# hyunlord/hnm_recommendation

Measured on AMD Instinct MI355X. Metric: recommendations/sec (batched users, K=12) at 1/2/4/8 MI355X; % HBM roofline, higher is better.
Workload: dtype f16+f32; 1 GPU; ncf: BASELINE configs[1] NeuralCF dim=64, full H&M shape, batch=4096 users/rank, K=12; users=1371980, items=105542, batch_per_rank=4096, k=12, parallelism=single, model=NeuralCF, mf_dim=64, weights=init, scan=certified f16 pre-filter + exact fp32 re-scoring (ncf_cert.hip)

## Files before the change

hnm_recommendation_amd/_lib.py:

```python
from __future__ import annotations

import ctypes as C
import os
import threading
import weakref

import torch

PKG = os.path.dirname(os.path.abspath(__file__))
LIB_PATH = os.environ.get("HNM_LIB_PATH") or os.path.join(PKG, "libhnm_mi355x.so")

HNM_OK, HNM_EINVAL, HNM_EOOB, HNM_EHIP, HNM_ENOMEM, HNM_EUNSUPPORTED, HNM_ECOLL = 0, -1, -2, -3, -4, -5, -6

_p = C.c_void_p
_i64 = C.c_int64
_i32 = C.c_int32
_f32 = C.c_float


class NcfWeights(C.Structure):
    _fields_ = [("gmf_user", _p), ("gmf_item", _p), ("mlp_user", _p), ("mlp_item", _p),
                ("w1", _p), ("b1", _p), ("w2", _p), ("b2", _p), ("wp", _p), ("bp", _p),
                ("num_users", _i64), ("num_items", _i64), ("mf", _i32), ("h0", _i32),
                ("h1", _i32), ("h2", _i32), ("item_proj", _p)]
# ... 160 lines not shown
        if _lib is not None:
            return _lib
        if not os.path.exists(path):
            raise RuntimeError(
                f"{path} is missing: the MI355X HIP library was not built "
                "(run `python -m hnm_recommendation_amd.build`). There is no CPU fallback.")
        lib = C.CDLL(path)
        for name, (res, args) in _SIGS.items():
            fn = getattr(lib, name, None)
            if fn is None:
                continue
            fn.restype = res
            fn.argtypes = args
        if lib.hnm_abi_version() != 1:
            raise RuntimeError("libhnm_mi355x ABI version mismatch")
        _lib = lib
        return lib


def fn(name):
    lib = load()
    f = getattr(lib, name, None)
    if f is None:
        raise RuntimeError(f"{name} is not exported by {LIB_PATH}")
    return f


def check(status: int, what: str = ""):
    if status == HNM_OK:
        return
    msg = load().hnm_last_error().decode(errors="replace")
    if status == HNM_EOOB:
        raise IndexError(msg)
    if status in (HNM_EINVAL, HNM_EUNSUPPORTED):
        raise ValueError(f"{what}: {msg}")
    raise RuntimeError(f"{what}: {msg} (status {status})")


def call(name: str, *args):
    check(fn(name)(*args), name)


def call_weighted(name: str, at: int, w, *args):
    if w is not None:
        name, args = name.replace("_f32", "_weighted_f32"), (*args[:at], ptr(w), *args[at:])
    check(fn(name)(*args), name)


def require_gpu(*tensors):
    for t in tensors:
        if t is None:
            continue
        on_gpu = t.type == "cuda" if isinstance(t, torch.device) else (
            isinstance(t, torch.Tensor) and t.is_cuda)
        if not on_gpu:
            raise RuntimeError(
                "hnm_recommendation_amd runs on an AMD Instinct GPU (MI355X) through its HIP "
                "library; move the module and its inputs to a GPU device (model.to('cuda')). "
                "There is no CPU path.")


def _dev_index(device) -> int:
    dev = torch.device(device)
    return dev.index if dev.index is not None else torch.cuda.current_device()


_opts: dict = {}


class _Ctx:
    __slots__ = ("handle", "device", "__weakref__")

    def __init__(self, device: int):
        h = _p()
        check(fn("hnm_ctx_create")(device, C.byref(h)), "hnm_ctx_create")
        self.handle, self.device = h, device

    def __del__(self):
        h, self.handle = self.handle, None
        lib = _lib
        if h and lib is not None:
            try:
                lib.hnm_ctx_destroy(h)
            except Exception:
                pass


def _thread_ctx(idx: int) -> "_Ctx":
    slots = getattr(_tls, "ctxs", None)
    if slots is None:
        slots = _tls.ctxs = {}
    c = slots.get(idx)
    if c is None:
        c = _Ctx(idx)
        with _lock:
            for opt, val in _opts.get(idx, {}).items():
                check(fn("hnm_ctx_set_option")(c.handle, int(opt), int(val)), "hnm_ctx_set_option")
            _live.add(c)
        slots[idx] = c
    return c


def _device_ctxs(idx: int):
    with _lock:
        return [c for c in list(_live) if c.device == idx and c.handle]


def live_contexts(device=None) -> int:
    if device is None:
        with _lock:
            return sum(1 for c in list(_live) if c.handle)
    return len(_device_ctxs(_dev_index(device)))


def ctx(device: torch.device):
    idx = _dev_index(device)
    c = _thread_ctx(idx)
    stream = torch.cuda.current_stream(idx).cuda_stream
    check(fn("hnm_ctx_set_stream")(c.handle, _p(stream)), "hnm_ctx_set_stream")
    return c.handle


def abort_pending(device):
    check(fn("hnm_ctx_abort_pending")(ctx(device)), "hnm_ctx_abort_pending")


def sync_check(device):
    check(fn("hnm_ctx_check")(ctx(device)), "hnm_ctx_check")


TIME_SCORE, TIME_SPMM = 1, 2


def enable_timing(device, on=True):
    check(fn("hnm_ctx_enable_timing")(ctx(device), int(on)), "hnm_ctx_enable_timing")


def kernel_timing(device):
    t = C.c_double()
    n = _i64()
    check(fn("hnm_ctx_timing")(ctx(device), C.byref(t), C.byref(n)), "hnm_ctx_timing")
    return t.value, n.value


HNM_OPT_PREFILTER = 1
HNM_OPT_STATS = 3
HNM_OPT_STRIDED = 4
HNM_OPT_DEEP_MFMA = 5
HNM_OPT_LINEAR_MFMA = 6
HNM_OPT_NCF_TABLES = 7
HNM_OPT_SCAN_SHAPE = 8
HNM_OPT_SCAN_PIPE = 9
HNM_OPT_SCAN_SPARSE = 10


def set_option(device, option, value):
    idx = _dev_index(device)
    ctx(device)
    with _lock:
        _opts.setdefault(idx, {})[int(option)] = int(value)
    for c in _device_ctxs(idx):
        check(fn("hnm_ctx_set_option")(c.handle, int(option), int(value)), "hnm_ctx_set_option")


def set_prefilter(device, on=True):
    set_option(device, HNM_OPT_PREFILTER, int(bool(on)))


def prefilter_stats(device, reset=False, extended=False):
    ctx(device)
    n = {"gate": 6, "cascade": 7}.get(extended, 4) if extended else 3
    tot = [0] * n
    for c in _device_ctxs(_dev_index(device)):
        out = (_i64 * n)()
        check(fn("hnm_ctx_prefilter_stats_ex")(c.handle, out, n, int(reset)),
              "hnm_ctx_prefilter_stats_ex")
        for j in range(n):
            tot[j] += int(out[j])
    return tuple(tot)


def ptr(t):
    return None if t is None else _p(t.data_ptr())
```

hnm_recommendation_amd/csrc/api.hip:

```cpp
#include <stdlib.h>
#include <string.h>

#include "hnm_device.h"
#include "hnm_internal.h"
#include "linear_mfma.h"

static thread_local char g_err[512] = "";

void hnm_set_error(const char* fmt, ...) {
  va_list ap;
  va_start(ap, fmt);
  vsnprintf(g_err, sizeof(g_err), fmt, ap);
  va_end(ap);
}

extern "C" int hnm_abi_version(void) { return HNM_ABI_VERSION; }
extern "C" const char* hnm_last_error(void) { return g_err; }

extern "C" hnm_status hnm_ctx_create(int device, hnm_ctx** out) {
  HNM_REQUIRE(out, HNM_EINVAL, "hnm_ctx_create: out is NULL");
  int ndev = 0;
  HNM_HIP_CHECK(hipGetDeviceCount(&ndev));
  HNM_REQUIRE(device >= 0 && device < ndev, HNM_EINVAL, "hnm_ctx_create: no device %d (%d visible)",
              device, ndev);
  const HnmDeviceGuard guard(device);
  hnm_ctx* c = (hnm_ctx*)calloc(1, sizeof(hnm_ctx));
  HNM_REQUIRE(c, HNM_ENOMEM, "hnm_ctx_create: out of host memory");
  c->device = device;
  c->stream = 0;
  hipDeviceProp_t prop;
  if (hipGetDeviceProperties(&prop, device) == hipSuccess) c->num_cus = prop.multiProcessorCount;
  if (c->num_cus <= 0) c->num_cus = 256;
  c->prefilter = 1;
  c->strided = 0;
  c->deep_mfma = 1;
#ifndef HNM_LINEAR_MFMA_DEFAULT
#define HNM_LINEAR_MFMA_DEFAULT 1
#endif
  c->linear_mfma = HNM_LINEAR_MFMA_DEFAULT;
  c->ncf_tables = 1;
  c->scan_shape = 1;
  c->scan_pipe = 1;
  c->scan_sparse = 1;
  if (hipMalloc((void**)&c->err_dev, 128) != hipSuccess) {
    free(c);
    hnm_set_error("hnm_ctx_create: hipMalloc of the error word failed");
    return HNM_ENOMEM;
  }
  HNM_HIP_CHECK(hipMemset(c->err_dev, 0, 128));
  HNM_HIP_CHECK(hipEventCreateWithFlags(&c->chain_ev, hipEventDisableTiming));
  HNM_HIP_CHECK(hipStreamCreateWithFlags(&c->side, hipStreamNonBlocking));
  HNM_HIP_CHECK(hipEventCreateWithFlags(&c->side_in, hipEventDisableTiming));
  HNM_HIP_CHECK(hipEventCreateWithFlags(&c->side_out, hipEventDisableTiming));
  static_assert(8 + HNM_STATS_N * sizeof(unsigned long long) <= 128, "error word + counters");
  c->stats_dev = reinterpret_cast<unsigned long long*>(reinterpret_cast<char*>(c->err_dev) + 8);
  *out = c;
  return HNM_OK;
}

extern "C" hnm_status hnm_ctx_destroy(hnm_ctx* ctx) {
  HNM_CTX_DEVICE(ctx);
  if (!ctx) return HNM_OK;
  (void)hipDeviceSynchronize();
  for (int i = 0; i < ctx->cap; ++i) {
    (void)hipEventDestroy(ctx->ev0[i]);
    (void)hipEventDestroy(ctx->ev1[i]);
  }
  free(ctx->ev0);
  free(ctx->ev1);
  hnm_rccl_release(ctx);
  if (ctx->ws) (void)hipFree(ctx->ws);
  if (ctx->err_dev) (void)hipFree(ctx->err_dev);
  (void)hipEventDestroy(ctx->chain_ev);
  (void)hipEventDestroy(ctx->side_in);
  (void)hipEventDestroy(ctx->side_out);
  (void)hipStreamDestroy(ctx->side);
  free(ctx);
  return HNM_OK;
}

extern "C" hnm_status hnm_ctx_set_stream(hnm_ctx* ctx, void* s) {
  HNM_CTX_DEVICE(ctx);
  HNM_REQUIRE(ctx, HNM_EINVAL, "ctx is NULL");
  const hipStream_t ns = (hipStream_t)s;
  if (ns == ctx->stream) return HNM_OK;
  HNM_HIP_CHECK(hipEventRecord(ctx->chain_ev, ctx->stream));
  HNM_HIP_CHECK(hipStreamWaitEvent(ns, ctx->chain_ev, 0));
  ctx->stream = ns;
  return HNM_OK;
}

extern "C" hnm_status hnm_ctx_abort_pending(hnm_ctx* ctx) {
  HNM_CTX_DEVICE(ctx);
  HNM_REQUIRE(ctx, HNM_EINVAL, "ctx is NULL");
  ctx->pend.kind = 0;
  return HNM_OK;
}

extern "C" hnm_status hnm_ctx_set_option(hnm_ctx* ctx, int option, int64_t value) {
  HNM_CTX_DEVICE(ctx);
  HNM_REQUIRE(ctx, HNM_EINVAL, "ctx is NULL");
  switch (option) {
    case HNM_OPT_PREFILTER:
      ctx->prefilter = value != 0;
      return HNM_OK;
    case HNM_OPT_STATS:
      ctx->stats_on = value != 0;
      return HNM_OK;
    case HNM_OPT_STRIDED:
      ctx->strided = value != 0;
      return HNM_OK;
    case HNM_OPT_DEEP_MFMA:
      ctx->deep_mfma = value != 0;
      return HNM_OK;
    case HNM_OPT_LINEAR_MFMA:
      ctx->linear_mfma = value != 0;
      return HNM_OK;
    case HNM_OPT_NCF_TABLES:
      ctx->ncf_tables = value != 0;
      return HNM_OK;
    case HNM_OPT_SCAN_SHAPE:
      ctx->scan_shape = value != 0;
      return HNM_OK;
    case HNM_OPT_SCAN_PIPE:
      ctx->scan_pipe = value != 0;
      return HNM_OK;
    case HNM_OPT_SCAN_SPARSE:
      ctx->scan_sparse = value != 0;
      return HNM_OK;
    default:
      hnm_set_error("hnm_ctx_set_option: unknown option %d", option);
      return HNM_EINVAL;
  }
}

extern "C" hnm_status hnm_ctx_prefilter_stats(hnm_ctx* ctx, int64_t* out, int reset) {
  HNM_CTX_DEVICE(ctx);
  return hnm_ctx_prefilter_stats_ex(ctx, out, 3, reset);
}

extern "C" hnm_status hnm_ctx_prefilter_stats_ex(hnm_ctx* ctx, int64_t* out, int n, int reset) {
  HNM_CTX_DEVICE(ctx);
  HNM_REQUIRE(ctx && out, HNM_EINVAL, "ctx/out is NULL");
  HNM_REQUIRE(n >= 1 && n <= HNM_STATS_N, HNM_EINVAL, "prefilter_stats: 1 <= n <= %d", HNM_STATS_N);
  int prev = -1;
  HNM_HIP_CHECK(hipGetDevice(&prev));
  struct Restore {
    int dev;
    ~Restore() { (void)hipSetDevice(dev); }
  } restore{prev};
  HNM_HIP_CHECK(hipSetDevice(ctx->device));
  HNM_HIP_CHECK(hipDeviceSynchronize());
  unsigned long long v[HNM_STATS_N];
  HNM_HIP_CHECK(hipMemcpy(v, ctx->stats_dev, sizeof(v), hipMemcpyDeviceToHost));
  for (int i = 0; i < n; ++i) out[i] = (int64_t)v[i];
  if (reset) HNM_HIP_CHECK(hipMemset(ctx->stats_dev, 0, sizeof(v)));
  return HNM_OK;
}

extern "C" hnm_status hnm_ctx_num_cus(hnm_ctx* ctx, int* out) {
  HNM_CTX_DEVICE(ctx);
  HNM_REQUIRE(ctx && out, HNM_EINVAL, "ctx/out is NULL");
  *out = ctx->num_cus;
  return HNM_OK;
}

hnm_status hnm_workspace(hnm_ctx* ctx, size_t bytes, void** out) {
  HNM_REQUIRE(!ctx->pend.kind, HNM_EINVAL,
              "a two-phase top-K call is open on this ctx: call its _finish first");
  bytes = hnm_align(bytes);
  if (bytes > ctx->ws_size) {
    HNM_HIP_CHECK(hipStreamSynchronize(ctx->stream));
    if (ctx->ws) HNM_HIP_CHECK(hipFree(ctx->ws));
    ctx->ws = nullptr;
    ctx->ws_size = 0;
    size_t want = hnm_align(bytes + bytes / 4);
    if (hipMalloc(&ctx->ws, want) != hipSuccess) {
      hnm_set_error("workspace: hipMalloc(%zu) failed", want);
      return HNM_ENOMEM;
    }
    ctx->ws_size = want;
  }
  *out = ctx->ws;
  return HNM_OK;
}

__global__ void fill_f32_kernel(float* __restrict__ p, int64_t n, float v) {
  const int64_t x = (int64_t)blockIdx.x * 256 + threadIdx.x;
  if (x < n) p[x] = v;
}

hnm_status hnm_fill_f32(hnm_ctx* ctx, float* p, int64_t n, float v) {
  if (n <= 0) return HNM_OK;
  hipLaunchKernelGGL(fill_f32_kernel, dim3((unsigned)hnm_cdiv(n, 256)), dim3(256), 0, ctx->stream,
                     p, n, v);
  HNM_LAUNCH_CHECK();
  return HNM_OK;
}

__global__ void trim_below_kernel(float* __restrict__ ov, int64_t* __restrict__ oi, int64_t n,
                                  int K, const float* __restrict__ lb) {
  const int64_t x = (int64_t)blockIdx.x * 256 + threadIdx.x;
  if (x >= n) return;
  if (ov[x] < lb[x / K]) {
    ov[x] = -__builtin_inff();
    oi[x] = -1;
  }
}

hnm_status hnm_topk_trim_below(hnm_ctx* ctx, float* ov, int64_t* oi, int64_t B, int K,
                               const float* lb) {
  if (B <= 0 || !ov || !oi || !lb) return HNM_OK;
  hipLaunchKernelGGL(trim_below_kernel, dim3((unsigned)hnm_cdiv(B * K, 256)), dim3(256), 0,
                     ctx->stream, ov, oi, B * K, K, lb);
  HNM_LAUNCH_CHECK();
  return HNM_OK;
}

extern "C" hnm_status hnm_ctx_reserve(hnm_ctx* ctx, size_t bytes) {
  HNM_CTX_DEVICE(ctx);
  HNM_REQUIRE(ctx, HNM_EINVAL, "ctx is NULL");
  void* p;
  return hnm_workspace(ctx, bytes, &p);
}

#define HNM_TIMER_PREALLOC 1024
static bool timer_grow(hnm_ctx* ctx, int ncap) {
  hipEvent_t* a = (hipEvent_t*)realloc(ctx->ev0, ncap * sizeof(hipEvent_t));
  if (a) ctx->ev0 = a;
  hipEvent_t* b = (hipEvent_t*)realloc(ctx->ev1, ncap * sizeof(hipEvent_t));
  if (b) ctx->ev1 = b;
  if (!a || !b) return false;
  for (int i = ctx->cap; i < ncap; ++i) {
    (void)hipEventCreate(&ctx->ev0[i]);
    (void)hipEventCreate(&ctx->ev1[i]);
  }
  ctx->cap = ncap;
  return true;
}

void hnm_timer_begin(hnm_ctx* ctx, int cls) {
  if (!(ctx->timing & cls)) return;
  if (ctx->nev == ctx->cap && !timer_grow(ctx, ctx->cap ? 2 * ctx->cap : 256)) {
    ctx->timing = 0;
    return;
  }
  (void)hipEventRecord(ctx->ev0[ctx->nev], ctx->stream);
}

void hnm_timer_end(hnm_ctx* ctx, int cls) {
  if (!(ctx->timing & cls) || ctx->nev >= ctx->cap) return;
  (void)hipEventRecord(ctx->ev1[ctx->nev], ctx->stream);
  ++ctx->nev;
}

extern "C" hnm_status hnm_ctx_enable_timing(hnm_ctx* ctx, int on) {
  HNM_CTX_DEVICE(ctx);
  HNM_REQUIRE(ctx, HNM_EINVAL, "ctx is NULL");
  if (on && ctx->cap < HNM_TIMER_PREALLOC && !timer_grow(ctx, HNM_TIMER_PREALLOC)) on = 0;
  ctx->timing = on;
  ctx->nev = 0;
  return HNM_OK;
}

extern "C" hnm_status hnm_ctx_timing(hnm_ctx* ctx, double* total_ms, int64_t* launches) {
  HNM_CTX_DEVICE(ctx);
  HNM_REQUIRE(ctx && total_ms && launches, HNM_EINVAL, "hnm_ctx_timing: NULL argument");
  HNM_HIP_CHECK(hipStreamSynchronize(ctx->stream));
  double t = 0.0;
  for (int i = 0; i < ctx->nev; ++i) {
    float ms = 0.f;
    HNM_HIP_CHECK(hipEventElapsedTime(&ms, ctx->ev0[i], ctx->ev1[i]));
    t += ms;
  }
  *total_ms = t;
  *launches = ctx->nev;
  ctx->nev = 0;
  return HNM_OK;
}

extern "C" hnm_status hnm_ctx_check(hnm_ctx* ctx) {
// ... 639 lines not shown
```

hnm_recommendation_amd/csrc/hnm_internal.h:

```cpp
#pragma once
#include <hip/hip_runtime.h>
#include <stdarg.h>
#include <stdint.h>
#include <stdio.h>

#include <algorithm>

#include "../../include/hnm.h"

struct hnm_ctx {
  int device;
  hipStream_t stream;
  hipEvent_t chain_ev;
  hipStream_t side;
  hipEvent_t side_in, side_out;
  void* ws;
  size_t ws_size;
  unsigned* err_dev;
  int num_cus;
  int timing;
  int nev;
  int cap;
  hipEvent_t* ev0;
  hipEvent_t* ev1;
  int prefilter;
  int strided;
  int deep_mfma;
  int linear_mfma;
  int ncf_tables;
  int scan_shape;
  int scan_pipe;
  int scan_sparse;
  void* comm;
  int comm_owned;
  unsigned long long* stats_dev;
  int stats_on;
  struct {
    int kind;
    int64_t B, I;
    int K;
    const void* ids;
    const void* items;
    int flags;
  } pend;
};
struct HnmDeviceGuard {
  int prev = -1;
  explicit HnmDeviceGuard(int device) {
    int cur = -1;
    if (device >= 0 && hipGetDevice(&cur) == hipSuccess && cur != device &&
        hipSetDevice(device) == hipSuccess)
      prev = cur;
  }
  ~HnmDeviceGuard() {
    if (prev >= 0) (void)hipSetDevice(prev);
  }
  HnmDeviceGuard(const HnmDeviceGuard&) = delete;
  HnmDeviceGuard& operator=(const HnmDeviceGuard&) = delete;
};
#define HNM_CTX_DEVICE(c) const HnmDeviceGuard hnm_device_guard_((c) ? (c)->device : -1)
#define HNM_STATS_N 7
#define HNM_PEND_NCF_CERT 1
#define HNM_PEND_NCF_EXACT 2
#define HNM_PEND_DOT_CERT 3
#define HNM_PEND_DOT_EXACT 4
#define HNM_PEND_STRIDED 1

#define HNM_TIME_SCORE 1
#define HNM_TIME_SPMM 2
void hnm_timer_begin(hnm_ctx* ctx, int cls);
void hnm_timer_end(hnm_ctx* ctx, int cls);

void hnm_set_error(const char* fmt, ...);
void hnm_rccl_release(hnm_ctx* ctx);

#define HNM_HIP_CHECK(expr)                                                        \
  do {                                                                             \
    hipError_t _e = (expr);                                                        \
    if (_e != hipSuccess) {                                                        \
      hnm_set_error("%s failed: %s (%s:%d)", #expr, hipGetErrorString(_e), __FILE__, \
                    __LINE__);                                                     \
      return HNM_EHIP;                                                             \
    }                                                                              \
  } while (0)

#define HNM_REQUIRE(cond, code, ...)  \
  do {                                \
    if (!(cond)) {                    \
      hnm_set_error(__VA_ARGS__);     \
      return (code);                  \
    }                                 \
  } while (0)

#define HNM_LAUNCH_CHECK()                                                          \
  do {                                                                              \
    hipError_t _e = hipGetLastError();                                              \
    if (_e != hipSuccess) {                                                         \
      hnm_set_error("kernel launch failed: %s (%s:%d)", hipGetErrorString(_e),      \
                    __FILE__, __LINE__);                                            \
      return HNM_EHIP;                                                              \
    }                                                                               \
  } while (0)

hnm_status hnm_workspace(hnm_ctx* ctx, size_t bytes, void** out);
hnm_status hnm_topk_rows_sort(hnm_ctx* ctx, const float* scores, int64_t ld, int64_t B,
                              int64_t I, const int64_t* mask_ptr, const int32_t* mask_idx, int k,
                              float* out_val, int64_t* out_idx);

static inline size_t hnm_align(size_t x, size_t a = 256) { return (x + a - 1) / a * a; }
__host__ __device__ static inline int64_t hnm_cdiv(int64_t a, int64_t b) { return (a + b - 1) / b; }

struct Partition {
  int np;
  int64_t ipp;
};
__host__ __device__ static inline Partition choose_partition(int64_t I, int64_t ublocks,
                                                             int num_cus, int64_t tile = 32,
                                                             int wg_per_cu = 2) {
  int64_t want = (int64_t)wg_per_cu * num_cus / (ublocks > 1 ? ublocks : 1);
  if (want < 1) want = 1;
  int64_t maxp = hnm_cdiv(I, 4 * tile);
  if (maxp < 1) maxp = 1;
  int64_t np = want < maxp ? want : maxp;
  int64_t ipp = hnm_cdiv(hnm_cdiv(I, np), tile) * tile;
  np = hnm_cdiv(I, ipp);
  return {(int)np, ipp};
}

static inline int64_t list_rows_grid(int64_t B, int64_t I, int num_cus) {
  int64_t best = 1;
  for (int64_t nb = 1; nb <= hnm_cdiv(B, 128); ++nb) {
    const int np = choose_partition(I, nb, num_cus).np;
    best = std::max<int64_t>(best, nb * np);
    if (np == 1) {
      best = std::max<int64_t>(best, hnm_cdiv(B, 128));
      break;
    }
  }
  return best;
}
static inline int64_t list_rows_slots(int64_t B, int64_t I, int num_cus) {
  int64_t best = 0;
  for (int64_t nb = 1; nb <= hnm_cdiv(B, 128); ++nb) {
    const int64_t n = std::min<int64_t>(B, nb * 128);
    best = std::max<int64_t>(best, n * choose_partition(I, nb, num_cus).np);
    if (choose_partition(I, nb, num_cus).np == 1) {
      best = std::max<int64_t>(best, B);
      break;
    }
  }
  return best;
}

hnm_status hnm_topk_rows_strided(hnm_ctx* ctx, const float* s, int64_t ld, int64_t B, int64_t I,
                                 const int64_t* mptr, const int32_t* midx, int K, float* ov,
                                 int64_t* oi, int64_t istride);
hnm_status hnm_sample_kth(hnm_ctx* ctx, const float* s, int64_t ld, int64_t B, int64_t Ns,
                          const int64_t* mptr, const int32_t* midx, int K, int64_t grp,
                          int64_t period, const int32_t* sidx, float* out,
                          const int* gate = nullptr);

hnm_status hnm_topk_merge_rows(hnm_ctx* ctx, const float* cv, const int32_t* ci, int64_t B,
                               int64_t G, int64_t gstride, int64_t bstride, int kc, int k,
                               float* ov, int64_t* oi, const int32_t* rows,
                               const int32_t* nrows, int64_t dyn_items = 0, int dyn_cus = 0);
hnm_status hnm_topk_merge_i32(hnm_ctx* ctx, const float* cv, const int32_t* ci, int64_t B,
                              int64_t G, int64_t gstride, int64_t bstride, int kc, int k,
                              float* ov, int64_t* oi);

hnm_status hnm_fill_f32(hnm_ctx* ctx, float* p, int64_t n, float v);
hnm_status hnm_topk_trim_below(hnm_ctx* ctx, float* ov, int64_t* oi, int64_t B, int K,
                               const float* lb);
```

hnm_recommendation_amd/csrc/ncf_cert_rescore.hip:

```cpp
#include <algorithm>

#include "ncf_cert_internal.h"

namespace {

#ifndef RESCORE_PERSIST
#define RESCORE_PERSIST 3
#endif
#ifndef RESCORE_BEST_FIRST_AB
#define RESCORE_BEST_FIRST_AB 96
#endif
constexpr int RESCORE_BEST_FIRST = RESCORE_BEST_FIRST_AB;
template <bool DEEP>
__global__ __launch_bounds__(256, DEEP ? 2 : 3) void ncf_rescore_kernel(
    NcfTabs t, int mf, const float* __restrict__ W2, int h1, int h2, const float* __restrict__ b2,
    const float* __restrict__ wm, const float* __restrict__ bp, int64_t B,
    const int* __restrict__ flag, const int* __restrict__ cnt, const int32_t* __restrict__ buf,
    const float* __restrict__ bufd, const float* __restrict__ tau, const float* __restrict__ Eu,
    const float* __restrict__ Au, const float* __restrict__ Cu, const CertParams* __restrict__ prm,
    int NP, int capp, int K, int short_ok, float* __restrict__ ov, int64_t* __restrict__ oi,
    int32_t* __restrict__ ovf_rows, int32_t* __restrict__ ovf_cnt,
    unsigned long long* __restrict__ stats, CertDeep dp, int64_t num_users) {
  constexpr int KS = 32;
  __shared__ int stg[4][96];
  __shared__ float w3l[DEEP ? 16 * 64 : 1];
  __shared__ float b3l[16], wpl[DEEP ? 128 + 16 : 1];
  __shared__ float g0l[DEEP ? 4 : 1][64];
  __shared__ __attribute__((aligned(16))) float wgs[4][64];
  __shared__ __attribute__((aligned(16))) float b2l[32], wml[32];
  __shared__ int pref[4][CERT_MAX_NP + 1];
  __shared__ float w2l[KS * 64];
  __shared__ __attribute__((aligned(16))) float pl[4][64];
  const int tid = threadIdx.x, lane = tid & 63, wave = tid >> 6, h = lane >> 5, j = lane & 31;
  if (tid < 32) {
    b2l[tid] = tid < h2 ? b2[tid] : 0.f;
    wml[tid] = !DEEP && tid < h2 ? wm[tid] : 0.f;
  }
  for (int e = tid; e < KS * 64; e += 256) {
    const int s = e >> 6, jj = e & 31, k = 2 * s + ((e >> 5) & 1);
    const int row = DEEP ? 2 * ((jj & 3) + 4 * (jj >> 3)) + ((jj >> 2) & 1) : jj;
    w2l[e] = (row < h2 && k < h1) ? W2[row * h1 + k] : 0.f;
  }
  if constexpr (DEEP) {
    for (int e = tid; e < 16 * 64; e += 256) {
      const int s = e >> 6, jj = e & 31, k = 2 * s + ((e >> 5) & 1);
      const int m = (jj & 3) + 4 * (jj >> 3);
      w3l[e] = (((jj >> 2) & 1) == 0 && m < dp.h3 && k < h2) ? dp.W3[m * h2 + k] : 0.f;
    }
    if (tid < 16) b3l[tid] = tid < dp.h3 ? dp.b3[tid] : 0.f;
    for (int e = tid; e < mf + dp.h3; e += 256) wpl[e] = dp.wp[e];
  }
  __syncthreads();
  for (int64_t b = (int64_t)blockIdx.x * 4 + wave; b < B; b += (int64_t)gridDim.x * 4) {
    wgs[wave][lane] = t.WGu[b * 64 + lane];
    pl[wave][lane] = t.Pu[b * 64 + lane];
    const int c = lane < NP ? cnt[b * NP + lane] : 0;
    if constexpr (DEEP) {
      const int64_t uid = dp.ids[b];
      g0l[wave][lane] =
          (lane < mf && uid >= 0 && uid < num_users) ? dp.gmf_user[uid * mf + lane] : 0.f;
    }
    int incl = c;
#pragma unroll
    for (int o = 1; o < 64; o <<= 1) {
      const int v = __shfl_up(incl, o);
      if (lane >= o) incl += v;
    }
    if (lane == 0) pref[wave][0] = 0;
    if (lane < NP) pref[wave][lane + 1] = incl;
    __builtin_amdgcn_fence(__ATOMIC_RELEASE, "wavefront");
    __builtin_amdgcn_wave_barrier();
    __builtin_amdgcn_fence(__ATOMIC_ACQUIRE, "wavefront");
    const int n = hnm_readlane_i(incl, 63);
    const bool over = __ballot(c > capp) != 0;
    if (flag[b] || over || (n < K && !short_ok)) {
      if (lane == 0) {
        ovf_rows[atomicAdd(ovf_cnt, 1)] = (int32_t)b;
        if (stats) {
          atomicAdd(&stats[2], 1ull);
          if (b == 0) atomicAdd(&stats[0], (unsigned long long)B);
        }
      }
      continue;
    }
    const float bpv = bp[0];
    WaveTopK<1> L;
    L.init();
    const int32_t* rowbuf = buf + b * (int64_t)NP * capp;
    const float* rowd = bufd + b * (int64_t)NP * capp;
    auto slot = [&](int g) {
      int lo = 0, hi = NP;
      while (hi - lo > 1) {
        const int mid = (lo + hi) >> 1;
        if (pref[wave][mid] <= g) lo = mid;
        else hi = mid;
      }
      return (int64_t)lo * capp + (g - pref[wave][lo]);
    };
    auto cand = [&](int g) { return g < n ? rowbuf[slot(g)] : 0; };
    auto score_deep = [&](int item, bool ok) {
      float q[KS];
      const float* qrow = t.Qi + (int64_t)item * 64 + h * KS;
#pragma unroll
      for (int s4 = 0; s4 < KS / 4; ++s4) {
        const float4 v = *reinterpret_cast<const float4*>(qrow + 4 * s4);
        q[4 * s4] = v.x; q[4 * s4 + 1] = v.y; q[4 * s4 + 2] = v.z; q[4 * s4 + 3] = v.w;
      }
      f32x16 acc = {};
      typedef __attribute__((address_space(3))) const float* lds_ptr;
#pragma unroll
      for (int s = 0; s < KS; s += 4) {
        float w[4], pv[4];
        asm volatile("ds_read_b32 %0, %8\n\tds_read_b32 %1, %9\n\tds_read_b32 %2, %10\n\t"
                     "ds_read_b32 %3, %11\n\tds_read_b32 %4, %12\n\tds_read_b32 %5, %13\n\t"
                     "ds_read_b32 %6, %14\n\tds_read_b32 %7, %15\n\ts_waitcnt lgkmcnt(0)"
                     : "=&v"(w[0]), "=&v"(w[1]), "=&v"(w[2]), "=&v"(w[3]),
                       "=&v"(pv[0]), "=&v"(pv[1]), "=&v"(pv[2]), "=&v"(pv[3])
                     : "v"((unsigned)(uintptr_t)(lds_ptr)&w2l[s * 64 + lane]),
                       "v"((unsigned)(uintptr_t)(lds_ptr)&w2l[(s + 1) * 64 + lane]),
                       "v"((unsigned)(uintptr_t)(lds_ptr)&w2l[(s + 2) * 64 + lane]),
                       "v"((unsigned)(uintptr_t)(lds_ptr)&w2l[(s + 3) * 64 + lane]),
                       "v"((unsigned)(uintptr_t)(lds_ptr)&pl[wave][h * KS + s]),
                       "v"((unsigned)(uintptr_t)(lds_ptr)&pl[wave][h * KS + s + 1]),
                       "v"((unsigned)(uintptr_t)(lds_ptr)&pl[wave][h * KS + s + 2]),
                       "v"((unsigned)(uintptr_t)(lds_ptr)&pl[wave][h * KS + s + 3]));
#pragma unroll
        for (int e = 0; e < 4; ++e) acc = mfma32x32x2(w[e], fmaxf(pv[e] + q[s + e], 0.f), acc);
      }
      f32x16 a3 = {};
#pragma unroll
      for (int s = 0; s < 16; ++s)
        a3 = mfma32x32x2(w3l[s * 64 + lane], fmaxf(acc[s] + b2l[2 * s + h], 0.f), a3);
      float sc = 0.f;
      if (h == 0 && ok) {
        const float* grow = dp.gmf_item + (int64_t)item * mf;
        for (int j4 = 0; j4 < mf; j4 += 4) {
          const float4 gv = *reinterpret_cast<const float4*>(grow + j4);
          sc = fmaf(wpl[j4], g0l[wave][j4] * gv.x, sc);
          sc = fmaf(wpl[j4 + 1], g0l[wave][j4 + 1] * gv.y, sc);
          sc = fmaf(wpl[j4 + 2], g0l[wave][j4 + 2] * gv.z, sc);
          sc = fmaf(wpl[j4 + 3], g0l[wave][j4 + 3] * gv.w, sc);
        }
#pragma unroll
        for (int m = 0; m < 16; ++m)
          if (m < dp.h3) sc = fmaf(wpl[mf + m], fmaxf(a3[m] + b3l[m], 0.f), sc);
      }
      L.offer(sc + bp[0], item, ok && h == 0, K);
    };
    auto score_item = [&](int item, bool ok) {
      if constexpr (DEEP) {
        score_deep(item, ok);
        return;
      }
      float gm = 0.f;
      const float* grow = t.G + (int64_t)item * t.ldg;
      const int glast = (int)t.ldg - 4;
#pragma unroll
      for (int half = 0; half < 2; ++half) {
        float4 gv[8];
#pragma unroll
        for (int q4 = 0; q4 < 8; ++q4)
          gv[q4] = *reinterpret_cast<const float4*>(grow + std::min(4 * (8 * half + q4), glast));
#pragma unroll
        for (int q4 = 0; q4 < 8; ++q4) {
          const int c4 = 8 * half + q4;
          const bool in = 4 * c4 < mf;
          const float2 wv = *reinterpret_cast<const float2*>(&wgs[wave][2 * c4]);
          const float2 wv1 = *reinterpret_cast<const float2*>(&wgs[wave][KS + 2 * c4]);
          gm = fmaf(wv1.x, in ? gv[q4].y : 0.f, fmaf(wv.x, in ? gv[q4].x : 0.f, gm));
          gm = fmaf(wv1.y, in ? gv[q4].w : 0.f, fmaf(wv.y, in ? gv[q4].z : 0.f, gm));
        }
      }
      float q[KS];
      const float* qrow = t.Qi + (int64_t)item * 64 + h * KS;
#pragma unroll
      for (int s4 = 0; s4 < KS / 4; ++s4) {
        const float4 v = *reinterpret_cast<const float4*>(qrow + 4 * s4);
        q[4 * s4] = v.x; q[4 * s4 + 1] = v.y; q[4 * s4 + 2] = v.z; q[4 * s4 + 3] = v.w;
      }
      f32x16 acc;
      float wmr[16];
#pragma unroll
      for (int r4 = 0; r4 < 4; ++r4) {
        const float4 bb = *reinterpret_cast<const float4*>(&b2l[8 * r4 + 4 * h]);
        const float4 ww = *reinterpret_cast<const float4*>(&wml[8 * r4 + 4 * h]);
        acc[4 * r4] = bb.x; acc[4 * r4 + 1] = bb.y; acc[4 * r4 + 2] = bb.z; acc[4 * r4 + 3] = bb.w;
        wmr[4 * r4] = ww.x; wmr[4 * r4 + 1] = ww.y; wmr[4 * r4 + 2] = ww.z; wmr[4 * r4 + 3] = ww.w;
      }
      typedef __attribute__((address_space(3))) const float* lds_ptr;
#pragma unroll
      for (int s = 0; s < KS; s += 4) {
        float w[4], pv[4];
        asm volatile("ds_read_b32 %0, %8\n\tds_read_b32 %1, %9\n\tds_read_b32 %2, %10\n\t"
                     "ds_read_b32 %3, %11\n\tds_read_b32 %4, %12\n\tds_read_b32 %5, %13\n\t"
                     "ds_read_b32 %6, %14\n\tds_read_b32 %7, %15\n\ts_waitcnt lgkmcnt(0)"
                     : "=&v"(w[0]), "=&v"(w[1]), "=&v"(w[2]), "=&v"(w[3]),
                       "=&v"(pv[0]), "=&v"(pv[1]), "=&v"(pv[2]), "=&v"(pv[3])
                     : "v"((unsigned)(uintptr_t)(lds_ptr)&w2l[s * 64 + lane]),
                       "v"((unsigned)(uintptr_t)(lds_ptr)&w2l[(s + 1) * 64 + lane]),
                       "v"((unsigned)(uintptr_t)(lds_ptr)&w2l[(s + 2) * 64 + lane]),
                       "v"((unsigned)(uintptr_t)(lds_ptr)&w2l[(s + 3) * 64 + lane]),
                       "v"((unsigned)(uintptr_t)(lds_ptr)&pl[wave][h * KS + s]),
                       "v"((unsigned)(uintptr_t)(lds_ptr)&pl[wave][h * KS + s + 1]),
                       "v"((unsigned)(uintptr_t)(lds_ptr)&pl[wave][h * KS + s + 2]),
                       "v"((unsigned)(uintptr_t)(lds_ptr)&pl[wave][h * KS + s + 3]));
#pragma unroll
        for (int e = 0; e < 4; ++e) acc = mfma32x32x2(w[e], fmaxf(pv[e] + q[s + e], 0.f), acc);
      }
      float m4[4] = {0.f, 0.f, 0.f, 0.f};
#pragma unroll
      for (int r = 0; r < 16; ++r) m4[r & 3] = fmaf(fmaxf(acc[r], 0.f), wmr[r], m4[r & 3]);
      const float mlp = (m4[0] + m4[1]) + (m4[2] + m4[3]);
      const float tot = hnm_sum_halves(mlp + (h == 0 ? gm : 0.f));
      const float score = tot + bpv;
      L.offer(score, item, ok && h == 0, K);
    };
    int* st = stg[wave];
    int ns = 0, nscored = 0;
    float v63 = 0.f, t2 = 0.f;
    int i63 = 0;
    bool usable = false;
    const float tb = tau[b];
    const bool bf = n > RESCORE_BEST_FIRST;
    int ti = HNM_SENTINEL_IDX;
    if (bf) {
      float tv = -__builtin_inff();
      for (int c0 = 0; c0 < n; c0 += 64) {
        const int g = c0 + lane;
        const float d = g < n ? rowd[slot(g)] : -__builtin_inff();
        float v1 = d != d ? __builtin_inff() : d;
        int i1 = g < n ? g : HNM_SENTINEL_IDX;
        const float c63 = hnm_readlane_f(tv, 63);
        const int c63i = hnm_readlane_i(ti, 63);
        if (__ballot(hnm_better(v1, i1, c63, c63i))) hnm_sort128(tv, ti, v1, i1);
      }
      v63 = hnm_readlane_f(tv, 63);
      i63 = hnm_readlane_i(ti, 63);
    }
    for (int phase = bf ? 0 : 2; phase < (bf ? 2 : 3); ++phase) {
      if (phase == 0) {
        st[lane] = ti;
        ns = 64;
      }
      if (phase == 1) {
        const float thr = L.thr_v;
        const float unit = prm->unit;
        const float scale = unit * (prm->c0 + Au[b] + prm->Bmax + Cu[b] * prm->Dmax);
        t2 = (thr - bpv) * unit - Eu[b] - 2.f * 3.814697265625e-06f * scale;
        t2 -= fabsf(t2) * 1.9073486328125e-06f;
        usable = __builtin_isfinite(t2);
      }
      for (int c0 = 0; c0 < (phase == 0 ? 1 : n); c0 += 64) {
        if (phase != 0) {
          const int g = c0 + lane;
          bool keep = g < n;
          if (keep && phase == 1) {
            const float d = rowd[slot(g)];
            const bool top = !hnm_better(v63, i63, d != d ? __builtin_inff() : d, g);
            keep = !top && (!usable || !(d + tb < t2));
          }
          const uint64_t m = __ballot(keep);
          if (keep) st[ns + __popcll(m & ((1ull << lane) - 1))] = g;
          ns += __popcll(m);
        }
        __builtin_amdgcn_fence(__ATOMIC_RELEASE, "wavefront");
        __builtin_amdgcn_wave_barrier();
        __builtin_amdgcn_fence(__ATOMIC_ACQUIRE, "wavefront");
        const bool last = phase == 0 || c0 + 64 >= n;
        while (ns >= 32 || (last && ns > 0)) {
          const int nv = ns < 32 ? ns : 32;
          score_item(cand(st[j < nv ? j : 0]), j < nv);
          nscored += nv;
          const int rest = ns - nv;
          const int mv = lane < rest ? st[32 + lane] : 0;
          __builtin_amdgcn_wave_barrier();
          if (lane < rest) st[lane] = mv;
          __builtin_amdgcn_fence(__ATOMIC_RELEASE, "wavefront");
          __builtin_amdgcn_wave_barrier();
          __builtin_amdgcn_fence(__ATOMIC_ACQUIRE, "wavefront");
          ns = rest;
        }
      }
    }
    if (stats && lane == 0) {
      atomicAdd(&stats[1], (unsigned long long)nscored);
      if (b == 0) atomicAdd(&stats[0], (unsigned long long)B);
    }
    L.store(ov ? ov + b * K : nullptr, oi + b * K, K);
  }
}

template <bool DEEP>
void launch_rescore(hnm_ctx* ctx, const hnm_ncf_weights* w, const NcfTabs& t, int64_t B,
                    const CertPlan& pl, int K, int short_ok, float* ov, int64_t* oi,
                    const CertDeep& dv) {
  const CertWs& x = pl.ws;
  const int64_t rgrid = std::min<int64_t>(hnm_cdiv(B, 4), (int64_t)RESCORE_PERSIST * ctx->num_cus);
  hipLaunchKernelGGL(ncf_rescore_kernel<DEEP>, dim3((unsigned)rgrid), dim3(256), 0, ctx->stream, t,
                     w->mf, w->w2, w->h1, w->h2, w->b2, w->wp + w->mf, w->bp, B, x.flag, x.cnt,
                     x.buf, x.bufd, x.tau, x.Eu, x.Au, x.Cu, x.prm, pl.sh.part.np, pl.sh.capp, K,
                     short_ok, ov, oi, x.ovf_rows, x.ovf_cnt,
                     ctx->stats_on ? ctx->stats_dev : nullptr, dv, w->num_users);
}

}

void cert_launch_rescore(hnm_ctx* ctx, const hnm_ncf_weights* w, const NcfTabs& t, int64_t B,
                         const CertPlan& pl, int K, int short_ok, float* ov, int64_t* oi,
                         const CertDeep* dp) {
  if (dp) launch_rescore<true>(ctx, w, t, B, pl, K, short_ok, ov, oi, *dp);
  else launch_rescore<false>(ctx, w, t, B, pl, K, short_ok, ov, oi, CertDeep{});
}
```

include/hnm.h:

```cpp
#ifndef HNM_H_
#define HNM_H_

#include <stddef.h>
#include <stdint.h>

#ifdef __cplusplus
extern "C" {
#endif

#define HNM_ABI_VERSION 1

typedef int32_t hnm_status;
enum {
  HNM_OK = 0,
  HNM_EINVAL = -1,
  HNM_EOOB = -2,
  HNM_EHIP = -3,
  HNM_ENOMEM = -4,
  HNM_EUNSUPPORTED = -5,
  HNM_ECOLL = -6
};

typedef struct hnm_ctx hnm_ctx;
typedef struct hnm_spmm_plan hnm_spmm_plan;

int hnm_abi_version(void);
const char* hnm_last_error(void);

hnm_status hnm_ctx_create(int device, hnm_ctx** out);
hnm_status hnm_ctx_destroy(hnm_ctx* ctx);
hnm_status hnm_ctx_set_stream(hnm_ctx* ctx, void* hip_stream);
hnm_status hnm_ctx_reserve(hnm_ctx* ctx, size_t bytes);
hnm_status hnm_ctx_check(hnm_ctx* ctx);
hnm_status hnm_ctx_num_cus(hnm_ctx* ctx, int* out);
hnm_status hnm_ctx_abort_pending(hnm_ctx* ctx);
enum { HNM_OPT_PREFILTER = 1,
       HNM_OPT_STATS = 3,
       HNM_OPT_STRIDED = 4,
       HNM_OPT_DEEP_MFMA = 5   ,
       HNM_OPT_LINEAR_MFMA = 6  };
#define HNM_OPT_NCF_TABLES 7
#define HNM_OPT_SCAN_SHAPE 8
#define HNM_OPT_SCAN_PIPE 9
#define HNM_OPT_SCAN_SPARSE 10
hnm_status hnm_ctx_set_option(hnm_ctx* ctx, int option, int64_t value);
hnm_status hnm_ctx_prefilter_stats(hnm_ctx* ctx, int64_t* out, int reset);
hnm_status hnm_ctx_prefilter_stats_ex(hnm_ctx* ctx, int64_t* out, int n, int reset);
hnm_status hnm_ctx_enable_timing(hnm_ctx* ctx, int mask);
hnm_status hnm_ctx_timing(hnm_ctx* ctx, double* total_ms, int64_t* launches);

hnm_status hnm_gather_rows_f32(hnm_ctx* ctx, const float* table, int64_t rows, int64_t ld,
                               int d, const int64_t* ids, int64_t n, float* out,
                               int64_t ldo);

hnm_status hnm_linear_rows_f32(hnm_ctx* ctx, const float* X, int64_t ldx, const int64_t* ids,
                               int64_t x_rows, int64_t M, int K, const float* W,
                               int64_t ldw, const float* bias, int N, float* Y, int64_t ldy,
                               int pair_permute);

hnm_status hnm_dot_topk_f32(hnm_ctx* ctx, const float* user_tab, int64_t num_users,
                            int64_t ldu, const int64_t* user_ids, int64_t B,
                            const float* item_tab, int64_t num_items, int64_t ldi, int d,
                            const float* user_bias, const float* item_bias,
                            const float* const_bias, const int64_t* mask_ptr,
                            const int32_t* mask_idx, int k, float* out_val,
                            int64_t* out_idx);
hnm_status hnm_dot_topk_begin_f32(hnm_ctx* ctx, const float* user_tab, int64_t num_users,
                                  int64_t ldu, const int64_t* user_ids, int64_t B,
                                  const float* item_tab, int64_t num_items, int64_t ldi, int d,
                                  const float* user_bias, const float* item_bias,
                                  const float* const_bias, const int64_t* mask_ptr,
                                  const int32_t* mask_idx, int k, float* lower_bound);
hnm_status hnm_dot_topk_begin_lists_f32(hnm_ctx* ctx, const float* user_tab, int64_t num_users,
                                        int64_t ldu, const int64_t* user_ids, int64_t B,
                                        const float* item_tab, int64_t num_items, int64_t ldi,
                                        int d, const float* user_bias, const float* item_bias,
                                        const float* const_bias, const int64_t* mask_ptr,
                                        const int32_t* mask_idx, int k, float* lower_lists);
hnm_status hnm_dot_topk_finish_f32(hnm_ctx* ctx, const float* user_tab, int64_t num_users,
                                   int64_t ldu, const int64_t* user_ids, int64_t B,
                                   const float* item_tab, int64_t num_items, int64_t ldi, int d,
                                   const float* user_bias, const float* item_bias,
                                   const float* const_bias, const int64_t* mask_ptr,
                                   const int32_t* mask_idx, int k, const float* lower_bound,
                                   int short_ok, float* out_val, int64_t* out_idx);
hnm_status hnm_dot_prefilter_debug_f32(hnm_ctx* ctx, const float* user_tab, int64_t num_users,
                                       int64_t ldu, const int64_t* user_ids, int64_t B,
                                       const float* item_tab, int64_t num_items, int64_t ldi,
                                       int d, const float* user_bias, const float* item_bias,
                                       const float* const_bias, float* approx, int64_t lda,
                                       float* bound);
hnm_status hnm_dot_scores_f32(hnm_ctx* ctx, const float* user_tab, int64_t num_users,
                              int64_t ldu, const int64_t* user_ids, int64_t B,
                              const float* item_tab, int64_t num_items, int64_t ldi, int d,
                              const float* user_bias, const float* item_bias,
                              const float* const_bias, float* out, int64_t ldo);

hnm_status hnm_pair_dot_f32(hnm_ctx* ctx, const float* user_tab, int64_t num_users,
                            int64_t ldu, const float* item_tab, int64_t num_items, int64_t ldi,
                            int d, const int64_t* user_ids, const int64_t* item_ids, int64_t n,
                            const float* user_bias, const float* item_bias,
                            const float* const_bias, float* out);

typedef struct {
  const float* gmf_user;
  const float* gmf_item;
  const float* mlp_user;
  const float* mlp_item;
  const float* w1;
  const float* b1;
  const float* w2;
  const float* b2;
  const float* wp;
  const float* bp;
  int64_t num_users;
  int64_t num_items;
  int32_t mf;
  int32_t h0;
  int32_t h1;
  int32_t h2;
  const float* item_proj;
} hnm_ncf_weights;

hnm_status hnm_ncf_item_proj_f32(hnm_ctx* ctx, const hnm_ncf_weights* w, float* out);

hnm_status hnm_ncf_topk_f32(hnm_ctx* ctx, const hnm_ncf_weights* w, const int64_t* user_ids,
                            int64_t B, const int64_t* mask_ptr, const int32_t* mask_idx,
                            int k, float* out_val, int64_t* out_idx);
hnm_status hnm_ncf_topk_begin_f32(hnm_ctx* ctx, const hnm_ncf_weights* w,
                                  const int64_t* user_ids, int64_t B, const int64_t* mask_ptr,
                                  const int32_t* mask_idx, int k, float* lower_bound);
hnm_status hnm_ncf_topk_begin_lists_f32(hnm_ctx* ctx, const hnm_ncf_weights* w,
                                        const int64_t* user_ids, int64_t B,
                                        const int64_t* mask_ptr, const int32_t* mask_idx, int k,
                                        float* lower_lists);
hnm_status hnm_ncf_topk_finish_f32(hnm_ctx* ctx, const hnm_ncf_weights* w,
                                   const int64_t* user_ids, int64_t B, const int64_t* mask_ptr,
                                   const int32_t* mask_idx, int k, const float* lower_bound,
                                   int short_ok, float* out_val, int64_t* out_idx);
hnm_status hnm_ncf_scores_f32(hnm_ctx* ctx, const hnm_ncf_weights* w,
                              const int64_t* user_ids, int64_t B, float* out, int64_t ldo);
hnm_status hnm_ncf_prefilter_debug_f32(hnm_ctx* ctx, const hnm_ncf_weights* w,
                                       const int64_t* user_ids, int64_t B, float* approx,
                                       int64_t lda, float* bound);
hnm_status hnm_ncf_pair_scores_f32(hnm_ctx* ctx, const hnm_ncf_weights* w,
                                   const int64_t* user_ids, const int64_t* item_ids,
                                   int64_t n, float* out);

typedef struct {
  const float* gmf_user;
  const float* gmf_item;
  const float* mlp_user;
  const float* mlp_item;
  const float* w[8];
  const float* b[8];
  const float* wp;
  const float* bp;
  int64_t num_users;
  int64_t num_items;
  int32_t mf;
  int32_t nl;
  int32_t dims[9];
} hnm_ncf_deep_weights;

hnm_status hnm_ncf_deep_scores_f32(hnm_ctx* ctx, const hnm_ncf_deep_weights* w,
                                   const int64_t* user_ids, int64_t B, const int64_t* item_ids,
                                   float* out, int64_t ldo);
hnm_status hnm_ncf_deep_topk_f32(hnm_ctx* ctx, const hnm_ncf_deep_weights* w,
                                 const int64_t* user_ids, int64_t B, const int64_t* mask_ptr,
                                 const int32_t* mask_idx, int k, float* out_val,
                                 int64_t* out_idx);
hnm_status hnm_ncf_deep_route(hnm_ctx* ctx, const hnm_ncf_deep_weights* w, int* route);
hnm_status hnm_ncf_deep_prefilter_debug_f32(hnm_ctx* ctx, const hnm_ncf_deep_weights* w,
                                            const int64_t* user_ids, int64_t B, float* approx,
                                            int64_t lda, float* bound);

typedef struct {
  const float* deep_user;
  const float* deep_item;
  const float* w1;
  const float* b1;
  const float* bn1_w;
  const float* bn1_b;
  const float* bn1_mean;
  const float* bn1_var;
  const float* w2;
  const float* b2;
  const float* bn2_w;
  const float* bn2_b;
  const float* bn2_mean;
  const float* bn2_var;
  const float* w3;
  const float* b3;
  const float* bn3_w;
  const float* bn3_b;
  const float* bn3_mean;
  const float* bn3_var;
// ... 209 lines not shown
```

Measured before the change: 2.408 million users/s.

## Add occupancy-tuned non-deep rescore kernel variant with 4 blocks per CU

Adds an OCC template path for the non-deep NCF rescore kernel that raises launch bounds from 3 to 4 blocks per CU and sizes the persistent grid to match. The scoring body is rewritten to cut register pressure: it loads only half the G row per lane and swaps halves with permlane32_swap, does batched inline-asm LDS reads, and uses ds_bpermute for the prefix scan. The new path is on by default behind a new option. It aims to hide memory latency with more resident waves, at the cost of hand-written asm and possible spills under the tighter register budget.

```diff
diff --git a/hnm_recommendation_amd/_lib.py b/hnm_recommendation_amd/_lib.py
--- a/hnm_recommendation_amd/_lib.py
+++ b/hnm_recommendation_amd/_lib.py
@@ -336,6 +336,7 @@
 HNM_OPT_SCAN_SHAPE = 8
 HNM_OPT_SCAN_PIPE = 9
 HNM_OPT_SCAN_SPARSE = 10
+HNM_OPT_RESCORE_OCC = 11
 
 
 def set_option(device, option, value):
diff --git a/hnm_recommendation_amd/csrc/api.hip b/hnm_recommendation_amd/csrc/api.hip
--- a/hnm_recommendation_amd/csrc/api.hip
+++ b/hnm_recommendation_amd/csrc/api.hip
@@ -42,6 +42,7 @@
   c->scan_shape = 1;
   c->scan_pipe = 1;
   c->scan_sparse = 1;
+  c->rescore_occ = 1;
   if (hipMalloc((void**)&c->err_dev, 128) != hipSuccess) {
     free(c);
     hnm_set_error("hnm_ctx_create: hipMalloc of the error word failed");
@@ -127,6 +128,9 @@
       return HNM_OK;
     case HNM_OPT_SCAN_SPARSE:
       ctx->scan_sparse = value != 0;
+      return HNM_OK;
+    case HNM_OPT_RESCORE_OCC:
+      ctx->rescore_occ = value != 0;
       return HNM_OK;
     default:
       hnm_set_error("hnm_ctx_set_option: unknown option %d", option);
diff --git a/hnm_recommendation_amd/csrc/hnm_internal.h b/hnm_recommendation_amd/csrc/hnm_internal.h
--- a/hnm_recommendation_amd/csrc/hnm_internal.h
+++ b/hnm_recommendation_amd/csrc/hnm_internal.h
@@ -31,6 +31,7 @@
   int scan_shape;
   int scan_pipe;
   int scan_sparse;
+  int rescore_occ;
   void* comm;
   int comm_owned;
   unsigned long long* stats_dev;
diff --git a/hnm_recommendation_amd/csrc/ncf_cert_rescore.hip b/hnm_recommendation_amd/csrc/ncf_cert_rescore.hip
--- a/hnm_recommendation_amd/csrc/ncf_cert_rescore.hip
+++ b/hnm_recommendation_amd/csrc/ncf_cert_rescore.hip
@@ -11,8 +11,23 @@
 #define RESCORE_BEST_FIRST_AB 96
 #endif
 constexpr int RESCORE_BEST_FIRST = RESCORE_BEST_FIRST_AB;
-template <bool DEEP>
-__global__ __launch_bounds__(256, DEEP ? 2 : 3) void ncf_rescore_kernel(
+template <int S>
+__device__ __forceinline__ void rescore_lds4(unsigned wa, unsigned pa, float (&w)[4], f32x4& pv) {
+  asm volatile("ds_read_b32 %0, %5 offset:%7\n\tds_read_b32 %1, %5 offset:%8\n\t"
+               "ds_read_b32 %2, %5 offset:%9\n\tds_read_b32 %3, %5 offset:%10\n\t"
+               "ds_read_b128 %4, %6 offset:%11\n\ts_waitcnt lgkmcnt(0)"
+               : "=&v"(w[0]), "=&v"(w[1]), "=&v"(w[2]), "=&v"(w[3]), "=&v"(pv)
+               : "v"(wa), "v"(pa), "n"(S * 256), "n"((S + 1) * 256), "n"((S + 2) * 256),
+                 "n"((S + 3) * 256), "n"(S * 4));
+}
+__device__ __forceinline__ float rescore_from_upper(float x) {
+  const auto r = __builtin_amdgcn_permlane32_swap(__float_as_uint(x), __float_as_uint(x), false,
+                                                  false);
+  return __uint_as_float(r[1]);
+}
+
+template <bool DEEP, bool OCC>
+__global__ __launch_bounds__(256, DEEP ? 2 : (OCC ? 4 : 3)) void ncf_rescore_kernel(
     NcfTabs t, int mf, const float* __restrict__ W2, int h1, int h2, const float* __restrict__ b2,
     const float* __restrict__ wm, const float* __restrict__ bp, int64_t B,
     const int* __restrict__ flag, const int* __restrict__ cnt, const int32_t* __restrict__ buf,
@@ -31,7 +46,8 @@
   __shared__ int pref[4][CERT_MAX_NP + 1];
   __shared__ float w2l[KS * 64];
   __shared__ __attribute__((aligned(16))) float pl[4][64];
-  const int tid = threadIdx.x, lane = tid & 63, wave = tid >> 6, h = lane >> 5, j = lane & 31;
+  const int tid = threadIdx.x, lane0 = tid & 63;
+  const int wave = OCC ? __builtin_amdgcn_readfirstlane(tid >> 6) : tid >> 6;
   if (tid < 32) {
     b2l[tid] = tid < h2 ? b2[tid] : 0.f;
     wml[tid] = !DEEP && tid < h2 ? wm[tid] : 0.f;
@@ -52,6 +68,9 @@
   }
   __syncthreads();
   for (int64_t b = (int64_t)blockIdx.x * 4 + wave; b < B; b += (int64_t)gridDim.x * 4) {
+    int lane = lane0;
+    if constexpr (OCC) asm volatile("" : "+v"(lane));
+    const int h = lane >> 5, j = lane & 31;
     wgs[wave][lane] = t.WGu[b * 64 + lane];
     pl[wave][lane] = t.Pu[b * 64 + lane];
     const int c = lane < NP ? cnt[b * NP + lane] : 0;
@@ -63,7 +82,8 @@
     int incl = c;
 #pragma unroll
     for (int o = 1; o < 64; o <<= 1) {
-      const int v = __shfl_up(incl, o);
+      const int v =
+          OCC ? __builtin_amdgcn_ds_bpermute((lane - o) << 2, incl) : __shfl_up(incl, o);
       if (lane >= o) incl += v;
     }
     if (lane == 0) pref[wave][0] = 0;
@@ -147,9 +167,81 @@
       }
       L.offer(sc + bp[0], item, ok && h == 0, K);
     };
+    auto score_occ = [&](int item, bool ok) {
+      int hh = h, mfv = mf;
+      asm volatile("" : "+v"(hh), "+s"(mfv));
+      const float* grow = t.G + (int64_t)item * t.ldg;
+      const int glast = (int)t.ldg - 4;
+      float4 gv[8];
+#pragma unroll
+      for (int q4 = 0; q4 < 8; ++q4)
+        gv[q4] = *reinterpret_cast<const float4*>(grow + std::min(4 * (8 * hh + q4), glast));
+      float q[KS];
+      const float* qrow = t.Qi + (int64_t)item * 64 + hh * KS;
+#pragma unroll
+      for (int s4 = 0; s4 < KS / 4; ++s4) {
+        const float4 v = *reinterpret_cast<const float4*>(qrow + 4 * s4);
+        q[4 * s4] = v.x; q[4 * s4 + 1] = v.y; q[4 * s4 + 2] = v.z; q[4 * s4 + 3] = v.w;
+      }
+      float gm = 0.f;
+#pragma unroll
+      for (int half = 0; half < 2; ++half) {
+#pragma unroll
+        for (int q4 = 0; q4 < 8; ++q4) {
+          const int c4 = 8 * half + q4;
+          const bool in = 4 * c4 < mfv;
+          float4 g = gv[q4];
+          if (half == 1) {
+            g.x = rescore_from_upper(g.x); g.y = rescore_from_upper(g.y);
+            g.z = rescore_from_upper(g.z); g.w = rescore_from_upper(g.w);
+          }
+          const float2 wv = *reinterpret_cast<const float2*>(&wgs[wave][2 * c4]);
+          const float2 wv1 = *reinterpret_cast<const float2*>(&wgs[wave][KS + 2 * c4]);
+          gm = fmaf(wv1.x, in ? g.y : 0.f, fmaf(wv.x, in ? g.x : 0.f, gm));
+          gm = fmaf(wv1.y, in ? g.w : 0.f, fmaf(wv.y, in ? g.z : 0.f, gm));
+          if ((q4 & 3) == 3) __builtin_amdgcn_sched_barrier(0);
+        }
+      }
+      f32x16 acc;
+#pragma unroll
+      for (int r4 = 0; r4 < 4; ++r4) {
+        const float4 bb = *reinterpret_cast<const float4*>(&b2l[8 * r4 + 4 * hh]);
+        acc[4 * r4] = bb.x; acc[4 * r4 + 1] = bb.y; acc[4 * r4 + 2] = bb.z; acc[4 * r4 + 3] = bb.w;
+      }
+      typedef __attribute__((address_space(3))) const float* lds_ptr;
+      const unsigned wa = (unsigned)(uintptr_t)(lds_ptr)&w2l[32 * hh + j];
+      const unsigned pa = (unsigned)(uintptr_t)(lds_ptr)&pl[wave][hh * KS];
+#define RESCORE_STEP4(S)                                                                      \
+  {                                                                                           \
+    float w[4];                                                                               \
+    f32x4 pv;                                                                                 \
+    rescore_lds4<S>(wa, pa, w, pv);                                                           \
+    _Pragma("unroll") for (int e = 0; e < 4; ++e)                                             \
+        acc = mfma32x32x2(w[e], fmaxf(pv[e] + q[S + e], 0.f), acc);                           \
+  }
+      RESCORE_STEP4(0) RESCORE_STEP4(4) RESCORE_STEP4(8) RESCORE_STEP4(12)
+      RESCORE_STEP4(16) RESCORE_STEP4(20) RESCORE_STEP4(24) RESCORE_STEP4(28)
+#undef RESCORE_STEP4
+      float m4[4] = {0.f, 0.f, 0.f, 0.f};
+#pragma unroll
+      for (int r4 = 0; r4 < 4; ++r4) {
+        const float4 ww = *reinterpret_cast<const float4*>(&wml[8 * r4 + 4 * hh]);
+        m4[0] = fmaf(fmaxf(acc[4 * r4], 0.f), ww.x, m4[0]);
+        m4[1] = fmaf(fmaxf(acc[4 * r4 + 1], 0.f), ww.y, m4[1]);
+        m4[2] = fmaf(fmaxf(acc[4 * r4 + 2], 0.f), ww.z, m4[2]);
+        m4[3] = fmaf(fmaxf(acc[4 * r4 + 3], 0.f), ww.w, m4[3]);
+      }
+      const float mlp = (m4[0] + m4[1]) + (m4[2] + m4[3]);
+      const float tot = hnm_sum_halves(mlp + (h == 0 ? gm : 0.f));
+      L.offer(tot + bpv, item, ok && h == 0, K);
+    };
     auto score_item = [&](int item, bool ok) {
       if constexpr (DEEP) {
         score_deep(item, ok);
+        return;
+      }
+      if constexpr (OCC) {
+        score_occ(item, ok);
         return;
       }
       float gm = 0.f;
@@ -290,15 +382,16 @@
   }
 }
 
-template <bool DEEP>
+template <bool DEEP, bool OCC>
 void launch_rescore(hnm_ctx* ctx, const hnm_ncf_weights* w, const NcfTabs& t, int64_t B,
                     const CertPlan& pl, int K, int short_ok, float* ov, int64_t* oi,
                     const CertDeep& dv) {
   const CertWs& x = pl.ws;
-  const int64_t rgrid = std::min<int64_t>(hnm_cdiv(B, 4), (int64_t)RESCORE_PERSIST * ctx->num_cus);
-  hipLaunchKernelGGL(ncf_rescore_kernel<DEEP>, dim3((unsigned)rgrid), dim3(256), 0, ctx->stream, t,
-                     w->mf, w->w2, w->h1, w->h2, w->b2, w->wp + w->mf, w->bp, B, x.flag, x.cnt,
-                     x.buf, x.bufd, x.tau, x.Eu, x.Au, x.Cu, x.prm, pl.sh.part.np, pl.sh.capp, K,
+  constexpr int per_cu = OCC ? 4 : RESCORE_PERSIST;
+  const int64_t rgrid = std::min<int64_t>(hnm_cdiv(B, 4), (int64_t)per_cu * ctx->num_cus);
+  hipLaunchKernelGGL((ncf_rescore_kernel<DEEP, OCC>), dim3((unsigned)rgrid), dim3(256), 0,
+                     ctx->stream, t, w->mf, w->w2, w->h1, w->h2, w->b2, w->wp + w->mf, w->bp, B,
+                     x.flag, x.cnt, x.buf, x.bufd, x.tau, x.Eu, x.Au, x.Cu, x.prm, pl.sh.part.np, pl.sh.capp, K,
                      short_ok, ov, oi, x.ovf_rows, x.ovf_cnt,
                      ctx->stats_on ? ctx->stats_dev : nullptr, dv, w->num_users);
 }
@@ -308,6 +401,8 @@
 void cert_launch_rescore(hnm_ctx* ctx, const hnm_ncf_weights* w, const NcfTabs& t, int64_t B,
                          const CertPlan& pl, int K, int short_ok, float* ov, int64_t* oi,
                          const CertDeep* dp) {
-  if (dp) launch_rescore<true>(ctx, w, t, B, pl, K, short_ok, ov, oi, *dp);
-  else launch_rescore<false>(ctx, w, t, B, pl, K, short_ok, ov, oi, CertDeep{});
-}
+  if (dp) launch_rescore<true, false>(ctx, w, t, B, pl, K, short_ok, ov, oi, *dp);
+  else if (ctx->rescore_occ)
+    launch_rescore<false, true>(ctx, w, t, B, pl, K, short_ok, ov, oi, CertDeep{});
+  else launch_rescore<false, false>(ctx, w, t, B, pl, K, short_ok, ov, oi, CertDeep{});
+}
diff --git a/include/hnm.h b/include/hnm.h
--- a/include/hnm.h
+++ b/include/hnm.h
@@ -43,6 +43,7 @@
 #define HNM_OPT_SCAN_SHAPE 8
 #define HNM_OPT_SCAN_PIPE 9
 #define HNM_OPT_SCAN_SPARSE 10
+#define HNM_OPT_RESCORE_OCC 11
 hnm_status hnm_ctx_set_option(hnm_ctx* ctx, int option, int64_t value);
 hnm_status hnm_ctx_prefilter_stats(hnm_ctx* ctx, int64_t* out, int reset);
 hnm_status hnm_ctx_prefilter_stats_ex(hnm_ctx* ctx, int64_t* out, int n, int reset);
```

Result: no change. 2.424 million users/s, median of 6 (+0.7%).
